# codelion/adaptive-classifier

Measured on NVIDIA H100. Metric: queries/sec predict() bert-base 128-tok, 1M x 768 prototypes, higher is better.
Workload: dtype f16

## Files before the change

### adaptive_classifier_b200/csrc/gemm_tc.cuh

```cuda
#pragma once
#include "common.cuh"

namespace ac {

constexpr int GEMM_BLOCK_M = 128;
constexpr int GEMM_BLOCK_N = 128;
constexpr int GEMM_BLOCK_K = 32;
constexpr int GEMM_KIND_TF32 = 0, GEMM_KIND_F16 = 1;
__host__ __device__ constexpr int gemm_block_k(int kind) { return kind == GEMM_KIND_F16 ? 64 : 32; }
constexpr int GEMM_STAGES = 4;
constexpr int GEMM_EPI_COLS = GEMM_BLOCK_N / 2;
constexpr int GEMM_EPI_WARPS = 8;
constexpr int GEMM_MMA_THREAD0 = 32 * GEMM_EPI_WARPS;
constexpr int GEMM_PRODUCER_THREAD = GEMM_MMA_THREAD0 + 128;
constexpr int GEMM_THREADS = GEMM_PRODUCER_THREAD + 128;
constexpr int GEMM_EPI_REGS = 160, GEMM_MMA_REGS = 160, GEMM_PRODUCER_REGS = 24;
static_assert(128 * GEMM_PRODUCER_REGS + 128 * GEMM_MMA_REGS + 256 * GEMM_EPI_REGS <= 65536, "register split exceeds the file");
constexpr int GEMM_A_STAGE_BYTES = GEMM_BLOCK_M * 128;
constexpr int GEMM_B_STAGE_BYTES = GEMM_BLOCK_N * 128;
constexpr int GEMM_STAGE_BYTES = GEMM_A_STAGE_BYTES + GEMM_B_STAGE_BYTES;
constexpr int GEMM_ACC_LD = GEMM_BLOCK_N + 4;
constexpr int GEMM_ACC_BYTES = GEMM_BLOCK_M * GEMM_ACC_LD * 4;
constexpr int GEMM_EPI_STAGE_ROW_BYTES = 80;
constexpr int GEMM_EPI_STAGE_BYTES = 32 * GEMM_EPI_STAGE_ROW_BYTES;
constexpr int GEMM_SMEM_BYTES = GEMM_STAGES * GEMM_STAGE_BYTES + GEMM_ACC_BYTES + GEMM_EPI_WARPS * GEMM_EPI_STAGE_BYTES +
                                1024  + 256 ;
static_assert(GEMM_SMEM_BYTES <= 227 * 1024, "stage ring + accumulator tile do not fit");

#ifndef AC_MBAR_WATCHDOG
#define AC_MBAR_WATCHDOG 1
#endif

__device__ __forceinline__ void mbar_wait_guarded(uint64_t *bar, uint32_t parity) {
#if AC_MBAR_WATCHDOG
    uint32_t spins = 0;
    while (!mbar_try_wait(bar, parity)) {
        if (++spins > (1u << 26)) __trap();
    }
#else
    mbar_wait(bar, parity);
#endif
}

struct GemmTileInfo {
    int m0, n0;
    int tile_iter;
};

__device__ __forceinline__ int gemm_epi_chalf() { return ((threadIdx.x >> 5) >> 1) & 1; }

template <class Epi, bool kMFastest = false, int kKind = GEMM_KIND_TF32>
__global__ void __launch_bounds__(GEMM_THREADS, 1)
gemm_tc_kernel(const __grid_constant__ CUtensorMap tmap_a, const __grid_constant__ CUtensorMap tmap_b,
               int M, int N, int K, Epi epi) {
    if (epi.skip_kernel()) return;
    extern __shared__ uint8_t smem_raw[];
    uint8_t *smem = reinterpret_cast<uint8_t *>((reinterpret_cast<uintptr_t>(smem_raw) + 1023) & ~uintptr_t(1023));
    uint8_t *smem_a = smem;
    uint8_t *smem_b = smem + GEMM_STAGES * GEMM_A_STAGE_BYTES;
    float *acc_tile = reinterpret_cast<float *>(smem + GEMM_STAGES * GEMM_STAGE_BYTES);
    uint8_t *epi_stage = smem + GEMM_STAGES * GEMM_STAGE_BYTES + GEMM_ACC_BYTES;
    uint64_t *bars = reinterpret_cast<uint64_t *>(epi_stage + GEMM_EPI_WARPS * GEMM_EPI_STAGE_BYTES);
    uint64_t *full_bar = bars;
    uint64_t *empty_bar = bars + GEMM_STAGES;
    uint64_t *acc_full = bars + 2 * GEMM_STAGES;
    uint64_t *acc_empty = acc_full + 1;

    const int warp = threadIdx.x >> 5;
    const int lane = threadIdx.x & 31;
    const int tiles_m = (M + GEMM_BLOCK_M - 1) / GEMM_BLOCK_M;
    const int tiles_n = (N + GEMM_BLOCK_N - 1) / GEMM_BLOCK_N;
    const int num_tiles = tiles_m * tiles_n;
    constexpr int BK = gemm_block_k(kKind);
    const int num_kb = (K + BK - 1) / BK;
    const int my_tiles = (num_tiles - static_cast<int>(blockIdx.x) + static_cast<int>(gridDim.x) - 1) / static_cast<int>(gridDim.x);

    if (threadIdx.x == GEMM_PRODUCER_THREAD) {
        tma_prefetch_desc(&tmap_a);
        tma_prefetch_desc(&tmap_b);
        for (int s = 0; s < GEMM_STAGES; ++s) {
            mbar_init(&full_bar[s], 1);
            mbar_init(&empty_bar[s], 4);
        }
        mbar_init(acc_full, 128);
        mbar_init(acc_empty, 32 * GEMM_EPI_WARPS);
        fence_mbar_init();
    }
    __syncthreads();

    if (threadIdx.x >= GEMM_PRODUCER_THREAD) {
        setmaxnreg_dec<GEMM_PRODUCER_REGS>();
        if (threadIdx.x == GEMM_PRODUCER_THREAD) {
            int stage = 0;
            uint32_t phase = 0;
            for (int tile = blockIdx.x; tile < num_tiles; tile += gridDim.x) {
                const int m0 = (kMFastest ? tile % tiles_m : tile / tiles_n) * GEMM_BLOCK_M;
                const int n0 = (kMFastest ? tile / tiles_m : tile % tiles_n) * GEMM_BLOCK_N;
                for (int kb = 0; kb < num_kb; ++kb) {
                    mbar_wait_guarded(&empty_bar[stage], phase ^ 1);
                    mbar_arrive_expect_tx(&full_bar[stage], GEMM_STAGE_BYTES);
                    tma_load_2d(smem_a + stage * GEMM_A_STAGE_BYTES, &tmap_a, &full_bar[stage], kb * BK, m0);
                    tma_load_2d(smem_b + stage * GEMM_B_STAGE_BYTES, &tmap_b, &full_bar[stage], kb * BK, n0);
                    if (++stage == GEMM_STAGES) { stage = 0; phase ^= 1; }
                }
            }
        }
        return;
    }

    if (threadIdx.x >= GEMM_MMA_THREAD0) {
        setmaxnreg_inc<GEMM_MMA_REGS>();
        const uint64_t a_desc0 = wgmma_desc_sw128(smem_u32(smem_a));
        const uint64_t b_desc0 = wgmma_desc_sw128(smem_u32(smem_b));
        int stage = 0;
        uint32_t phase = 0;
        for (int it = 0; it < my_tiles; ++it) {
            float acc0[64], acc1[64];
#pragma unroll
            for (int j = 0; j < 64; ++j) { acc0[j] = 0.f; acc1[j] = 0.f; }
            int prev_stage = -1;
            for (int kb = 0; kb < num_kb; ++kb) {
                mbar_wait_guarded(&full_bar[stage], phase);
                const uint64_t a_desc = a_desc0 + stage * (GEMM_A_STAGE_BYTES >> 4);
                const uint64_t b_desc = b_desc0 + stage * (GEMM_B_STAGE_BYTES >> 4);
                wgmma_fence();
#pragma unroll
                for (int k = 0; k < 4; ++k) {
                    if (kKind == GEMM_KIND_F16) {
                        wgmma_m64n128_f16(acc0, a_desc + 2 * k, b_desc + 2 * k, 1u);
                        wgmma_m64n128_f16(acc1, a_desc + 512 + 2 * k, b_desc + 2 * k, 1u);
                    } else {
                        wgmma_m64n128_tf32(acc0, a_desc + 2 * k, b_desc + 2 * k, 1u);
                        wgmma_m64n128_tf32(acc1, a_desc + 512 + 2 * k, b_desc + 2 * k, 1u);
                    }
                }
                wgmma_commit();
                wgmma_wait<1>();
                __syncwarp();
                if (prev_stage >= 0 && lane == 0) mbar_arrive(&empty_bar[prev_stage]);
                prev_stage = stage;
                if (++stage == GEMM_STAGES) { stage = 0; phase ^= 1; }
            }
            wgmma_wait<0>();
            __syncwarp();
            if (lane == 0) mbar_arrive(&empty_bar[prev_stage]);

            mbar_wait_guarded(acc_empty, (it & 1) ^ 1);
            wgmma_store_acc(acc0, acc_tile, GEMM_ACC_LD);
            wgmma_store_acc(acc1, acc_tile + 64 * GEMM_ACC_LD, GEMM_ACC_LD);
            mbar_arrive(acc_full);
        }
        return;
    }

    setmaxnreg_inc<GEMM_EPI_REGS>();
    const int wg = warp >> 2;
    const int q = 2 * wg + (warp & 1);
    const int chalf = gemm_epi_chalf();
    typename Epi::State est;
    epi.begin_cta(est, q, lane);
    const float *acc_row = acc_tile + (q * 32 + lane) * GEMM_ACC_LD;
    for (int it = 0; it < my_tiles; ++it) {
        const int tile = static_cast<int>(blockIdx.x) + it * static_cast<int>(gridDim.x);
        GemmTileInfo ti;
        ti.m0 = (kMFastest ? tile % tiles_m : tile / tiles_n) * GEMM_BLOCK_M;
        ti.n0 = (kMFastest ? tile / tiles_m : tile % tiles_n) * GEMM_BLOCK_N;
        ti.tile_iter = it;
        const int row = ti.m0 + q * 32 + lane;
        const int c_lo = chalf * GEMM_EPI_COLS;
        constexpr int kDist = Epi::kPrefetchDist, kBufs = kDist + 1, kChunks = GEMM_EPI_COLS / 32;
#pragma unroll
        for (int d = 0; d < kDist; ++d)
            if (d < kChunks) epi.prefetch(est, ti, row, ti.n0 + c_lo + 32 * d, lane, d % kBufs);

        mbar_wait_guarded(acc_full, it & 1);
#pragma unroll (Epi::kUnrollChunks)
        for (int ci = 0; ci < kChunks; ++ci) {
            const int c = c_lo + 32 * ci;
            if (ci + kDist < kChunks) epi.prefetch(est, ti, row, ti.n0 + c + 32 * kDist, lane, (ci + kDist) % kBufs);
            float v[32];
            acc_row_ld32(acc_row + c, v);
            epi.tile(est, ti, row, ti.n0 + c, v, epi_stage + warp * GEMM_EPI_STAGE_BYTES, lane, ci % kBufs, acc_row + c);
        }
        mbar_arrive(acc_empty);
    }
    epi.end_cta(est, q, lane);
}

template <class Epi, bool kMFastest = false, int kKind = GEMM_KIND_TF32>
int launch_gemm_tc(const CUtensorMap &ta, const CUtensorMap &tb, int M, int N, int K, const Epi &epi,
                   cudaStream_t stream, int max_ctas = 0, int prof_cls = PROF_GEMM_LINEAR, double prof_bytes = 0.0) {
    auto kern = gemm_tc_kernel<Epi, kMFastest, kKind>;
    static bool attr_set[64] = {};
    int dev = 0;
    AC_CUDA(cudaGetDevice(&dev));
    if (dev < 0 || dev >= 64 || !attr_set[dev]) {
        AC_CUDA(cudaFuncSetAttribute(kern, cudaFuncAttributeMaxDynamicSharedMemorySize, GEMM_SMEM_BYTES));
        if (dev >= 0 && dev < 64) attr_set[dev] = true;
    }
    const int tiles = ((M + GEMM_BLOCK_M - 1) / GEMM_BLOCK_M) * ((N + GEMM_BLOCK_N - 1) / GEMM_BLOCK_N);
    int ctas = sm_count();
    if (max_ctas > 0 && max_ctas < ctas) ctas = max_ctas;
    if (tiles < ctas) ctas = tiles;
    if (ctas <= 0) return AC_OK;
    const int slot = prof_begin(prof_cls, 2.0 * M * static_cast<double>(N) * K, prof_bytes, stream);
    kern<<<ctas, GEMM_THREADS, GEMM_SMEM_BYTES, stream>>>(ta, tb, M, N, K, epi);
    prof_end(slot, stream);
    AC_LAUNCH_CHECK();
    return AC_OK;
}

}
```

Before: 18050.

## Stagger the two MMA accumulator halves so each epilogue half overlaps the next tile

```diff
diff --git a/adaptive_classifier_b200/csrc/gemm_tc.cuh b/adaptive_classifier_b200/csrc/gemm_tc.cuh
--- a/adaptive_classifier_b200/csrc/gemm_tc.cuh
+++ b/adaptive_classifier_b200/csrc/gemm_tc.cuh
@@ -42,6 +42,36 @@
 #endif
 }
 
+__device__ __forceinline__ void mbar_wait_mma(uint64_t *bar, uint32_t parity, bool &stuck) {
+#if AC_MBAR_WATCHDOG
+    uint32_t spins = 0;
+    while (!stuck && !mbar_try_wait(bar, parity)) {
+        if (++spins > (1u << 26)) stuck = true;
+    }
+#else
+    mbar_wait(bar, parity);
+#endif
+}
+__device__ __forceinline__ void gemm_wait_full(uint64_t *full_bar, int g, bool &stuck) {
+    mbar_wait_mma(&full_bar[g % GEMM_STAGES], (g / GEMM_STAGES) & 1, stuck);
+}
+template <int kKind>
+__device__ __forceinline__ void gemm_issue_kblock(float (&acc)[64], uint64_t a_desc0, uint64_t b_desc0, int g, int a_rows) {
+    const int s = g % GEMM_STAGES;
+    const uint64_t a_desc = a_desc0 + s * (GEMM_A_STAGE_BYTES >> 4) + a_rows;
+    const uint64_t b_desc = b_desc0 + s * (GEMM_B_STAGE_BYTES >> 4);
+    wgmma_fence();
+#pragma unroll
+    for (int k = 0; k < 4; ++k) {
+        if (kKind == GEMM_KIND_F16) wgmma_m64n128_f16(acc, a_desc + 2 * k, b_desc + 2 * k, 1u);
+        else wgmma_m64n128_tf32(acc, a_desc + 2 * k, b_desc + 2 * k, 1u);
+    }
+}
+__device__ __forceinline__ void gemm_release(uint64_t *empty_bar, int g, int lane) {
+    __syncwarp();
+    if (lane == 0) mbar_arrive(&empty_bar[g % GEMM_STAGES]);
+}
+
 struct GemmTileInfo {
     int m0, n0;
     int tile_iter;
@@ -64,7 +94,7 @@
     uint64_t *full_bar = bars;
     uint64_t *empty_bar = bars + GEMM_STAGES;
     uint64_t *acc_full = bars + 2 * GEMM_STAGES;
-    uint64_t *acc_empty = acc_full + 1;
+    uint64_t *acc_empty = acc_full + 2;
 
     const int warp = threadIdx.x >> 5;
     const int lane = threadIdx.x & 31;
@@ -82,8 +112,10 @@
             mbar_init(&full_bar[s], 1);
             mbar_init(&empty_bar[s], 4);
         }
-        mbar_init(acc_full, 128);
-        mbar_init(acc_empty, 32 * GEMM_EPI_WARPS);
+        for (int h = 0; h < 2; ++h) {
+            mbar_init(&acc_full[h], 128);
+            mbar_init(&acc_empty[h], 128);
+        }
         fence_mbar_init();
     }
     __syncthreads();
@@ -112,44 +144,51 @@
         setmaxnreg_inc<GEMM_MMA_REGS>();
         const uint64_t a_desc0 = wgmma_desc_sw128(smem_u32(smem_a));
         const uint64_t b_desc0 = wgmma_desc_sw128(smem_u32(smem_b));
-        int stage = 0;
-        uint32_t phase = 0;
+        const int last_kb = num_kb - 1;
+        int ga = 0, gb = 0;
+        bool stuck = false;
+        float acc0[64], acc1[64];
+#pragma unroll
+        for (int j = 0; j < 64; ++j) { acc0[j] = 0.f; acc1[j] = 0.f; }
         for (int it = 0; it < my_tiles; ++it) {
-            float acc0[64], acc1[64];
-#pragma unroll
-            for (int j = 0; j < 64; ++j) { acc0[j] = 0.f; acc1[j] = 0.f; }
-            int prev_stage = -1;
-            for (int kb = 0; kb < num_kb; ++kb) {
-                mbar_wait_guarded(&full_bar[stage], phase);
-                const uint64_t a_desc = a_desc0 + stage * (GEMM_A_STAGE_BYTES >> 4);
-                const uint64_t b_desc = b_desc0 + stage * (GEMM_B_STAGE_BYTES >> 4);
-                wgmma_fence();
-#pragma unroll
-                for (int k = 0; k < 4; ++k) {
-                    if (kKind == GEMM_KIND_F16) {
-                        wgmma_m64n128_f16(acc0, a_desc + 2 * k, b_desc + 2 * k, 1u);
-                        wgmma_m64n128_f16(acc1, a_desc + 512 + 2 * k, b_desc + 2 * k, 1u);
-                    } else {
-                        wgmma_m64n128_tf32(acc0, a_desc + 2 * k, b_desc + 2 * k, 1u);
-                        wgmma_m64n128_tf32(acc1, a_desc + 512 + 2 * k, b_desc + 2 * k, 1u);
-                    }
-                }
+            gemm_wait_full(full_bar, ga, stuck);
+            gemm_issue_kblock<kKind>(acc0, a_desc0, b_desc0, ga++, 0);
+            wgmma_commit();
+            if (it > 0) {
+                wgmma_wait<0>();
+                gemm_release(empty_bar, gb - 1, lane);
+                mbar_wait_mma(&acc_empty[1], it & 1, stuck);
+                wgmma_store_acc(acc1, acc_tile + 64 * GEMM_ACC_LD, GEMM_ACC_LD);
+                mbar_arrive(&acc_full[1]);
+#pragma unroll
+                for (int j = 0; j < 64; ++j) acc1[j] = 0.f;
+            }
+            for (int kb = 0; kb < last_kb; ++kb) {
+                gemm_issue_kblock<kKind>(acc1, a_desc0, b_desc0, gb++, 512);
+                wgmma_commit();
+                gemm_wait_full(full_bar, ga, stuck);
+                gemm_issue_kblock<kKind>(acc0, a_desc0, b_desc0, ga++, 0);
                 wgmma_commit();
                 wgmma_wait<1>();
-                __syncwarp();
-                if (prev_stage >= 0 && lane == 0) mbar_arrive(&empty_bar[prev_stage]);
-                prev_stage = stage;
-                if (++stage == GEMM_STAGES) { stage = 0; phase ^= 1; }
+                gemm_release(empty_bar, gb - 1, lane);
             }
-            wgmma_wait<0>();
-            __syncwarp();
-            if (lane == 0) mbar_arrive(&empty_bar[prev_stage]);
-
-            mbar_wait_guarded(acc_empty, (it & 1) ^ 1);
+            gemm_issue_kblock<kKind>(acc1, a_desc0, b_desc0, gb++, 512);
+            wgmma_commit();
+            wgmma_wait<1>();
+            mbar_wait_mma(&acc_empty[0], (it & 1) ^ 1, stuck);
             wgmma_store_acc(acc0, acc_tile, GEMM_ACC_LD);
+            mbar_arrive(&acc_full[0]);
+#pragma unroll
+            for (int j = 0; j < 64; ++j) acc0[j] = 0.f;
+        }
+        wgmma_wait<0>();
+        if (my_tiles > 0) {
+            gemm_release(empty_bar, gb - 1, lane);
+            mbar_wait_mma(&acc_empty[1], my_tiles & 1, stuck);
             wgmma_store_acc(acc1, acc_tile + 64 * GEMM_ACC_LD, GEMM_ACC_LD);
-            mbar_arrive(acc_full);
-        }
+            mbar_arrive(&acc_full[1]);
+        }
+        if (stuck) __trap();
         return;
     }
 
@@ -173,7 +212,7 @@
         for (int d = 0; d < kDist; ++d)
             if (d < kChunks) epi.prefetch(est, ti, row, ti.n0 + c_lo + 32 * d, lane, d % kBufs);
 
-        mbar_wait_guarded(acc_full, it & 1);
+        mbar_wait_guarded(&acc_full[wg], it & 1);
 #pragma unroll (Epi::kUnrollChunks)
         for (int ci = 0; ci < kChunks; ++ci) {
             const int c = c_lo + 32 * ci;
@@ -182,7 +221,7 @@
             acc_row_ld32(acc_row + c, v);
             epi.tile(est, ti, row, ti.n0 + c, v, epi_stage + warp * GEMM_EPI_STAGE_BYTES, lane, ci % kBufs, acc_row + c);
         }
-        mbar_arrive(acc_empty);
+        mbar_arrive(&acc_empty[wg]);
     }
     epi.end_cta(est, q, lane);
 }
```

New measurement: 18470, median of 6. 1.02x the previous value.
